# ibm-granite/dolomite-engine

Hardware: NVIDIA H100
Metric: tokens_per_sec (higher is better)
Workload: dtype bf16

## Files before the change

### dolomite_engine_b200/csrc/attention_bwd.cu

```cuda
#include "attention_common.cuh"
#include "../../include/dolomite_b200.h"

using namespace dolo;

namespace {

struct BwdParams {
    const float* lse;
    const float* delta;
    __nv_bfloat16* dqkv;
    int64_t row_stride;
    const int32_t* cu_seqlens;
    int n_docs;
    int64_t T;
    int n_groups, q_per_group, n_heads;
    float scale, scale_log2;
    int head_chunk;
    int head_chunk_q;
    int n_tile_slots;
    AttnDropout drop;
    const float* alibi_slopes;
};

constexpr int DELTA_TOK = 8;
__global__ void __launch_bounds__(256)
    attn_delta_kernel(const uint4* __restrict__ dout, const uint4* __restrict__ out, float* __restrict__ delta, int64_t T,
                      int n_heads, int vec_per_head) {
    extern __shared__ float part[];
    const int64_t t0 = int64_t(blockIdx.x) * DELTA_TOK;
    const int ntok = (T - t0) < DELTA_TOK ? int(T - t0) : DELTA_TOK;
    const int vec_per_tok = n_heads * vec_per_head;
    const int total = ntok * vec_per_tok;
    const uint4* a = dout + t0 * vec_per_tok;
    const uint4* b = out + t0 * vec_per_tok;
    for (int i = threadIdx.x; i < total; i += blockDim.x) {
        const uint4 x = __ldg(a + i), y = __ldg(b + i);
        float s = bf16_lo(x.x) * bf16_lo(y.x) + bf16_hi(x.x) * bf16_hi(y.x);
        s += bf16_lo(x.y) * bf16_lo(y.y) + bf16_hi(x.y) * bf16_hi(y.y);
        s += bf16_lo(x.z) * bf16_lo(y.z) + bf16_hi(x.z) * bf16_hi(y.z);
        s += bf16_lo(x.w) * bf16_lo(y.w) + bf16_hi(x.w) * bf16_hi(y.w);
        part[i] = s;
    }
    __syncthreads();
    for (int i = threadIdx.x; i < n_heads * DELTA_TOK; i += blockDim.x) {
        const int h = i / DELTA_TOK, tl = i - h * DELTA_TOK;
        if (tl < ntok) {
            const float* p = part + tl * vec_per_tok + h * vec_per_head;
            float s = 0.f;
            for (int k = 0; k < vec_per_head; ++k) s += p[k];
            delta[int64_t(h) * T + t0 + tl] = s;
        }
    }
}

constexpr int ATT_BWD_THREADS = 384;
constexpr int ATT_PRODUCER_REGS = 24;
constexpr int ATT_CONSUMER_REGS = 240;
static_assert(ATT_PRODUCER_REGS * 128 + 2 * ATT_CONSUMER_REGS * 128 <= 65536, "register file exceeded");

constexpr int BWD_QT = 64;

__device__ __forceinline__ void opaque(uint32_t& x) { asm volatile("" : "+r"(x)); }
__device__ __forceinline__ void mbar_spin(uint64_t* bar, uint32_t parity) {
    asm volatile("{\n\t.reg .pred P1;\n\tWAIT_%=:\n\tmbarrier.try_wait.parity.shared::cta.b64 P1, [%0], %1;\n\t@!P1 bra WAIT_%=;\n\t}"
                 ::"r"(smem_u32(bar)), "r"(parity)
                 : "memory");
}
__device__ __forceinline__ void mbar_arrive_lane0(uint64_t* bar, int lane) {
    asm volatile("{\n\t.reg .pred p;\n\tsetp.eq.s32 p, %1, 0;\n\t@p mbarrier.arrive.shared::cta.b64 _, [%0];\n\t}" ::"r"(smem_u32(bar)),
                 "r"(lane)
                 : "memory");
}
constexpr int QDO_STAGES = 4;

template <bool ALIBI, bool MASK>
__device__ __forceinline__ void bwd_p_ds(float (&st)[BWD_QT / 2], float (&dpt)[BWD_QT / 2], const float* ls, const float* ds,
                                         const BwdParams& p, const TileLoc& loc, int q0, int wc, const int (&kr)[2], int head,
                                         uint32_t head_key, bool drop) {
    const float slope = ALIBI ? __ldg(p.alibi_slopes + head) : 0.f;
#pragma unroll
    for (int h = 0; h < 2; ++h) {
        const float bias_r = ALIBI ? attn_alibi_bias(slope, kr[h]) * ATT_LOG2E : 0.f;
#pragma unroll
        for (int b = 0; b < BWD_QT / 8; ++b) {
            const float2 l = *reinterpret_cast<const float2*>(ls + 8 * b + wc);
            const float2 d = *reinterpret_cast<const float2*>(ds + 8 * b + wc);
            const float lse_c[2] = {l.x, l.y}, del_c[2] = {d.x, d.y};
#pragma unroll
            for (int e = 0; e < 2; ++e) {
                const int q = q0 + 8 * b + wc + e;
                const int i = 4 * b + 2 * h + e;
                const bool ok = !MASK || (q >= kr[h] && q < loc.doc_len);
                float pr;
                if constexpr (ALIBI)
                    pr = ok ? fast_exp2(fmaf(st[i], p.scale_log2, bias_r) - lse_c[e]) : 0.f;
                else
                    pr = ok ? fast_exp2(fmaf(st[i], p.scale_log2, -lse_c[e])) : 0.f;
                float dp = dpt[i];
                if (drop) {
                    const float z = attn_drop_scale(p.drop, head_key, loc.doc_start + q, loc.doc_start + kr[h]);
                    dp *= z;
                    st[i] = pr * z;
                } else {
                    st[i] = pr;
                }
                dpt[i] = p.scale * pr * (dp - del_c[e]);
            }
        }
    }
}

template <int HD, bool ALIBI>
__global__ void __launch_bounds__(ATT_BWD_THREADS, 1)
    attn_bwd_kernel(const __grid_constant__ CUtensorMap tq64, const __grid_constant__ CUtensorMap tqR,
                    const __grid_constant__ CUtensorMap to64, const __grid_constant__ CUtensorMap toR, const BwdParams p) {
    using CH = HeadChunks<HD>;
    constexpr int KV_BYTES = CH::tile_bytes(ATT_TILE);
    constexpr int QT_BYTES = CH::tile_bytes(BWD_QT);

    int cta_tile, group;
    attn_cta_order(p.head_chunk, p.n_tile_slots, cta_tile, group);
    const TileLoc loc = locate_tile(p.cu_seqlens, p.n_docs, cta_tile);
    if (!loc.valid) return;
    const int k0 = loc.tile * ATT_TILE;
    const int i0 = k0 / BWD_QT;
    const int n_qt = (loc.doc_len + BWD_QT - 1) / BWD_QT;
    const int n_i = n_qt - i0;
    const int n_steps = n_i * p.q_per_group;
    const int k_col = (group * (p.q_per_group + 2) + p.q_per_group) * HD;
    const int v_col = k_col + HD;

    extern __shared__ uint8_t smem_raw[];
    uint8_t* smem = smem_align_1024(smem_raw);
    uint8_t* sK = smem;
    uint8_t* sV = sK + KV_BYTES;
    uint8_t* sQ = sV + KV_BYTES;
    uint8_t* sO = sQ + QDO_STAGES * QT_BYTES;
    float* sL = reinterpret_cast<float*>(sO + QDO_STAGES * QT_BYTES);
    uint64_t* bars = reinterpret_cast<uint64_t*>(sL + QDO_STAGES * 2 * BWD_QT);
    uint64_t* kv_full = bars;
    uint64_t* qd_full = bars + 1;
    uint64_t* qd_empty = bars + 1 + QDO_STAGES;

    const int wg = threadIdx.x >> 7, warp = threadIdx.x >> 5, lane = threadIdx.x & 31;
    const float log2e = 1.4426950408889634f;

    if (threadIdx.x == 0) {
        tma_prefetch_desc(&tq64);
        tma_prefetch_desc(&to64);
        if (CH::REM > 0) {
            tma_prefetch_desc(&tqR);
            tma_prefetch_desc(&toR);
        }
        mbar_init(kv_full, 1);
        for (int i = 0; i < QDO_STAGES; ++i) {
            mbar_init(&qd_full[i], 1 + 32);
            mbar_init(&qd_empty[i], 8);
        }
        mbar_fence_init();
        mbar_expect_tx(kv_full, 2 * KV_BYTES);
        tma_load_chunked<HD, ATT_TILE>(sK, &tq64, &tqR, kv_full, k_col, loc.doc_start + k0);
        tma_load_chunked<HD, ATT_TILE>(sV, &tq64, &tqR, kv_full, v_col, loc.doc_start + k0);
    }
    __syncthreads();

    if (wg == 0) {
        setmaxnreg_dec<ATT_PRODUCER_REGS>();
        if (warp == 0) {
            if (elect_one()) {
                int s = 0;
                uint32_t ph = 0;
                for (int n = 0; n < n_steps; ++n) {
                    const int hl = n / n_i, qi = i0 + n % n_i;
                    const int q_col = (group * (p.q_per_group + 2) + hl) * HD;
                    mbar_wait(&qd_empty[s], ph ^ 1, 32);
                    mbar_expect_tx(&qd_full[s], 2 * QT_BYTES);
                    tma_load_chunked<HD, BWD_QT>(sQ + s * QT_BYTES, &tq64, &tqR, &qd_full[s], q_col,
                                                 loc.doc_start + qi * BWD_QT);
                    tma_load_chunked<HD, BWD_QT>(sO + s * QT_BYTES, &to64, &toR, &qd_full[s],
                                                 (group * p.q_per_group + hl) * HD, loc.doc_start + qi * BWD_QT);
                    if (++s == QDO_STAGES) s = 0, ph ^= 1;
                }
            }
        } else if (warp == 1) {
            int s = 0;
            uint32_t ph = 0;
            for (int n = 0; n < n_steps; ++n) {
                const int hl = n / n_i, qi = i0 + n % n_i;
                const int64_t row0 = int64_t(group * p.q_per_group + hl) * p.T + loc.doc_start;
                mbar_wait(&qd_empty[s], ph ^ 1, 33);
                float* ls = sL + s * 2 * BWD_QT;
#pragma unroll
                for (int r = lane; r < BWD_QT; r += 32) {
                    const int q = qi * BWD_QT + r;
                    ls[r] = q < loc.doc_len ? __ldg(p.lse + row0 + q) * log2e : 0.f;
                    ls[BWD_QT + r] = q < loc.doc_len ? __ldg(p.delta + row0 + q) : 0.f;
                }
                mbar_arrive(&qd_full[s]);
                if (++s == QDO_STAGES) s = 0, ph ^= 1;
            }
        }
        return;
    }

    setmaxnreg_inc<ATT_CONSUMER_REGS>();
    const int cw = wg - 1;
    const int n_steps_u = __shfl_sync(0xffffffffu, n_steps, 0);
    const int wr = (warp & 3) * 16 + (lane >> 2);
    const int wc = 2 * (lane & 3);
    const int kr[2] = {k0 + cw * 64 + wr, k0 + cw * 64 + wr + 8};
    const bool drop = p.drop.threshold != 0;
    const uint32_t sk0 = smem_u32(sK), sv0 = smem_u32(sV);

    float dv[HD / 2], dk[HD / 2];
#pragma unroll
    for (int i = 0; i < HD / 2; ++i) dv[i] = dk[i] = 0.f;
    float st[BWD_QT / 2], dpt[BWD_QT / 2];

    auto issue_ss = [&](int s) {
        const uint32_t sq = smem_u32(sQ + s * QT_BYTES), so = smem_u32(sO + s * QT_BYTES);
        uint32_t sk = sk0, sv = sv0;
        opaque(sk), opaque(sv);
        wgmma_fence();
#pragma unroll
        for (int c = 0; c < CH::NCHUNK; ++c) {
            const int w = CH::width(c);
            const uint32_t krow = CH::offset(c, ATT_TILE) + cw * 64 * 2 * w;
#pragma unroll
            for (int k = 0; k < w / 16; ++k) {
                wgmma_ss<BWD_QT, 0, 0>(st, chunk_desc_kmajor(sk + krow, w, k), chunk_desc_kmajor(sq + CH::offset(c, BWD_QT), w, k),
                                       (c != 0 || k != 0) ? 1u : 0u);
                wgmma_ss<BWD_QT, 0, 0>(dpt, chunk_desc_kmajor(sv + krow, w, k), chunk_desc_kmajor(so + CH::offset(c, BWD_QT), w, k),
                                       (c != 0 || k != 0) ? 1u : 0u);
            }
        }
        wgmma_commit();
    };

    mbar_spin(kv_full, 0);
    int s = 0;
    uint32_t ph = 0;
    for (int n = 0; n < n_steps_u; ++n) {
        const int hl = n / n_i, qi = i0 + n % n_i;
        const int head = group * p.q_per_group + hl;
        const int q0 = qi * BWD_QT;
        const uint32_t head_key = dropout_head_key(uint32_t(head), p.drop.key0, p.drop.key1);
        mbar_spin(&qd_full[s], ph);
        issue_ss(s);
        wgmma_wait<0>();
        reg_fence<BWD_QT / 2>(st);
        reg_fence<BWD_QT / 2>(dpt);

        const float* ls = sL + s * 2 * BWD_QT;
        if (qi <= i0 + cw || (qi + 1) * BWD_QT > loc.doc_len)
            bwd_p_ds<ALIBI, true>(st, dpt, ls, ls + BWD_QT, p, loc, q0, wc, kr, head, head_key, drop);
        else
            bwd_p_ds<ALIBI, false>(st, dpt, ls, ls + BWD_QT, p, loc, q0, wc, kr, head, head_key, drop);
        uint32_t pa[BWD_QT / 16][4], da[BWD_QT / 16][4];
#pragma unroll
        for (int kk = 0; kk < BWD_QT / 16; ++kk) {
            acc_to_a_frag(st, kk, pa[kk]);
            acc_to_a_frag(dpt, kk, da[kk]);
        }

        uint32_t sq = smem_u32(sQ + s * QT_BYTES), so = smem_u32(sO + s * QT_BYTES);
        opaque(sq), opaque(so);
        wgmma_fence();
#pragma unroll
        for (int c = 0; c < CH::NCHUNK; ++c) {
#pragma unroll
            for (int kk = 0; kk < BWD_QT / 16; ++kk) {
                if (CH::width(c) == 64) {
                    wgmma_rs<64, 1>(dv + CH::col(c) / 2, pa[kk], chunk_desc_mnmajor(so + CH::offset(c, BWD_QT), 64, kk), 1u);
                    wgmma_rs<64, 1>(dk + CH::col(c) / 2, da[kk], chunk_desc_mnmajor(sq + CH::offset(c, BWD_QT), 64, kk), 1u);
                } else {
                    constexpr int R = CH::REM ? CH::REM : 16;
                    wgmma_rs<R, 1>(dv + CH::col(c) / 2, pa[kk], chunk_desc_mnmajor(so + CH::offset(c, BWD_QT), R, kk), 1u);
                    wgmma_rs<R, 1>(dk + CH::col(c) / 2, da[kk], chunk_desc_mnmajor(sq + CH::offset(c, BWD_QT), R, kk), 1u);
                }
            }
        }
        wgmma_commit();
        wgmma_wait<0>();
        reg_fence<HD / 2>(dv);
        reg_fence<HD / 2>(dk);
        __syncwarp();
        mbar_arrive_lane0(&qd_empty[s], lane);
        if (++s == QDO_STAGES) s = 0, ph ^= 1;
    }

#pragma unroll
    for (int h = 0; h < 2; ++h) {
        if (kr[h] >= loc.doc_len) continue;
        __nv_bfloat16* row = p.dqkv + (loc.doc_start + int64_t(kr[h])) * p.row_stride;
#pragma unroll
        for (int b = 0; b < HD / 8; ++b) {
            *reinterpret_cast<uint32_t*>(row + k_col + 8 * b + wc) = pack_bf16(dk[4 * b + 2 * h], dk[4 * b + 2 * h + 1]);
            *reinterpret_cast<uint32_t*>(row + v_col + 8 * b + wc) = pack_bf16(dv[4 * b + 2 * h], dv[4 * b + 2 * h + 1]);
        }
    }
}

template <int HD, bool ALIBI>
int launch_bwd(const void* dout, const void* qkv, int64_t row_stride, const BwdParams& p, cudaStream_t st) {
    using CH = HeadChunks<HD>;
    CUtensorMap tq64, tqR, to64, toR;
    int rc = attn_make_maps<HD>(qkv, row_stride, p.T, &tq64, &tqR);
    if (rc) return rc;
    rc = attn_make_maps<HD>(dout, int64_t(p.n_heads) * HD, p.T, &to64, &toR);
    if (rc) return rc;
    constexpr int smem_bytes = 1024 + 2 * CH::tile_bytes(ATT_TILE) + 2 * QDO_STAGES * CH::tile_bytes(BWD_QT) +
                               QDO_STAGES * 2 * BWD_QT * 4 + 128;
    static_assert(smem_bytes <= 232448, "attention backward shared memory budget exceeded");
    auto kern = attn_bwd_kernel<HD, ALIBI>;
    static bool attr_set = false;
    if (!attr_set) {
        DOLO_CUDA_OK(cudaFuncSetAttribute(kern, cudaFuncAttributeMaxDynamicSharedMemorySize, smem_bytes));
        attr_set = true;
    }
    const int64_t max_tiles = (p.T + ATT_TILE - 1) / ATT_TILE + p.n_docs;
    DOLO_REQUIRE(max_tiles == p.n_tile_slots && max_tiles * p.n_groups < (1ll << 31), "attn_bwd: grid too large");
    dim3 grid((unsigned)(max_tiles * p.n_groups));
    kern<<<grid, ATT_BWD_THREADS, smem_bytes, st>>>(tq64, tqR, to64, toR, p);
    DOLO_LAUNCH_OK("attn_varlen_bwd");
    return DOLO_OK;
}

constexpr int DQ_KT = 64;
constexpr int KV_STAGES = 4;

template <bool ALIBI, bool MASK>
__device__ __forceinline__ void dq_ds(float (&sc)[DQ_KT / 2], const float (&dp)[DQ_KT / 2], const BwdParams& p,
                                      const TileLoc& loc, int j, int wc, const int (&qr)[2], const float (&lse_r)[2],
                                      const float (&del_r)[2], float slope, uint32_t head_key, bool drop) {
    if constexpr (ALIBI) {
#pragma unroll
        for (int b = 0; b < DQ_KT / 8; ++b)
#pragma unroll
            for (int e = 0; e < 2; ++e) {
                const int k = j * DQ_KT + 8 * b + wc + e;
                const float bl = attn_alibi_bias(slope, k) * ATT_LOG2E;
#pragma unroll
                for (int h = 0; h < 2; ++h) {
                    const int i = 4 * b + 2 * h + e;
                    const bool ok = !MASK || (k <= qr[h] && qr[h] < loc.doc_len);
                    const float pr = ok ? fast_exp2(fmaf(sc[i], p.scale_log2, bl) - lse_r[h]) : 0.f;
                    float d = dp[i];
                    if (drop) d *= attn_drop_scale(p.drop, head_key, loc.doc_start + qr[h], loc.doc_start + k);
                    sc[i] = p.scale * pr * (d - del_r[h]);
                }
            }
    } else {
#pragma unroll
        for (int h = 0; h < 2; ++h)
#pragma unroll
            for (int b = 0; b < DQ_KT / 8; ++b)
#pragma unroll
                for (int e = 0; e < 2; ++e) {
                    const int k = j * DQ_KT + 8 * b + wc + e;
                    const int i = 4 * b + 2 * h + e;
                    const bool ok = !MASK || (k <= qr[h] && qr[h] < loc.doc_len);
                    const float pr = ok ? fast_exp2(fmaf(sc[i], p.scale_log2, -lse_r[h])) : 0.f;
                    float d = dp[i];
                    if (drop) d *= attn_drop_scale(p.drop, head_key, loc.doc_start + qr[h], loc.doc_start + k);
                    sc[i] = p.scale * pr * (d - del_r[h]);
                }
    }
}

template <int HD, bool ALIBI>
__global__ void __launch_bounds__(ATT_BWD_THREADS, 1)
    attn_dq_kernel(const __grid_constant__ CUtensorMap tq64, const __grid_constant__ CUtensorMap tqR,
                   const __grid_constant__ CUtensorMap to64, const __grid_constant__ CUtensorMap toR, const BwdParams p) {
    using CH = HeadChunks<HD>;
    constexpr int Q_BYTES = CH::tile_bytes(ATT_TILE);
// ... 304 lines not shown
```

### dolomite_engine_b200/csrc/attention_common.cuh

```cuda
#pragma once
#include "common.cuh"
#include "wgmma.cuh"
#include "../../include/dolomite_b200.h"

namespace dolo {

constexpr int ATT_TILE = 128;

template <int HD>
struct HeadChunks {
    static_assert(HD % 16 == 0 && HD >= 16 && HD <= 128, "head_dim must be a multiple of 16 in [16, 128]");
    static constexpr int NC64 = HD / 64;
    static constexpr int REM = HD % 64;
    static_assert(REM == 0 || REM == 16 || REM == 32, "head_dim % 64 must be 0, 16 or 32");
    static constexpr int NCHUNK = NC64 + (REM ? 1 : 0);
    __host__ __device__ static constexpr int width(int c) { return c < NC64 ? 64 : REM; }
    __host__ __device__ static constexpr int col(int c) { return c * 64; }
    __host__ __device__ static constexpr int offset(int c, int rows) { return c * rows * 128; }
    __host__ __device__ static constexpr int tile_bytes(int rows) { return rows * HD * 2; }
};

__host__ __device__ constexpr uint32_t chunk_layout_type(int w) { return w == 64 ? 1u : (w == 32 ? 2u : 3u); }

__device__ __forceinline__ uint64_t chunk_desc_kmajor(uint32_t chunk_saddr, int w, int k16) {
    return gmma_desc(chunk_saddr + k16 * 32, 16, 16 * w, chunk_layout_type(w));
}
__device__ __forceinline__ uint64_t chunk_desc_mnmajor(uint32_t chunk_saddr, int w, int k16) {
    return gmma_desc(chunk_saddr + k16 * 32 * w, 16 * w, 16 * w, chunk_layout_type(w));
}

template <int HD, int ROWS>
__device__ __forceinline__ void tma_load_chunked(uint8_t* dst, const CUtensorMap* m64, const CUtensorMap* mR, uint64_t* bar,
                                                 int col0, int row0) {
    using CH = HeadChunks<HD>;
#pragma unroll
    for (int c = 0; c < CH::NCHUNK; ++c)
#pragma unroll
        for (int h = 0; h < ROWS / 64; ++h)
            tma_load_2d(dst + CH::offset(c, ROWS) + h * 64 * 2 * CH::width(c), c < CH::NC64 ? m64 : mR, bar,
                        col0 + CH::col(c), row0 + h * 64);
}

template <int HD>
int attn_make_maps(const void* base, int64_t ld, int64_t rows, CUtensorMap* m64, CUtensorMap* mR) {
    using CH = HeadChunks<HD>;
    uint64_t dims[2] = {uint64_t(ld), uint64_t(rows)};
    uint64_t strides[2] = {2, uint64_t(ld) * 2};
    uint32_t box[2] = {64, 64};
    int rc;
    if (CH::NC64 > 0) {
        rc = dolo_make_tmap(m64, base, 2, 2, dims, strides, box, DOLO_SW_128);
        if (rc) return rc;
    }
    if (CH::REM > 0) {
        box[0] = CH::REM;
        rc = dolo_make_tmap(mR, base, 2, 2, dims, strides, box, CH::REM == 32 ? DOLO_SW_64 : DOLO_SW_32);
        if (rc) return rc;
    }
    if (CH::NC64 == 0) *m64 = *mR;
    if (CH::REM == 0) *mR = *m64;
    return DOLO_OK;
}

struct AttnDropout {
    uint32_t threshold;
    float keep_scale;
    uint32_t key0, key1;
};
__device__ __forceinline__ float attn_drop_scale(const AttnDropout& d, uint32_t head_key, int q_tok, int k_tok) {
    return dropout_hash_qk(uint32_t(q_tok), uint32_t(k_tok), head_key) >= d.threshold ? d.keep_scale : 0.f;
}

__device__ __forceinline__ float attn_alibi_bias(float slope, int kpos) {
    return __bfloat162float(__float2bfloat16_rn(slope * float(kpos)));
}
constexpr float ATT_LOG2E = 1.4426950408889634f;
constexpr float ATT_LN2 = 0.6931471805599453f;

__device__ __forceinline__ void attn_cta_order(int chunk, int n_tile_slots, int& tile, int& head) {
    const int id = int(blockIdx.x);
    if (chunk <= 0) {
        tile = id % n_tile_slots;
        head = id / n_tile_slots;
        return;
    }
    const int per = n_tile_slots * chunk;
    const int c = id / per, r = id - c * per;
    tile = r / chunk;
    head = c * chunk + (r - tile * chunk);
}
inline int attn_head_chunk(int option, int n, int align) {
    if (option <= 0 || n <= 0) return 0;
    if (align < 1 || n % align != 0) align = 1;
    int best = 0;
    for (int c = align; c <= n; c += align)
        if (n % c == 0 && c <= (option > align ? option : align)) best = c;
    return best > 0 ? best : n;
}

struct TileLoc {
    int doc_start;
    int doc_len;
    int tile;
    bool valid;
};
__device__ __forceinline__ TileLoc locate_tile(const int32_t* __restrict__ cu, int n_docs, int ti) {
    TileLoc r{0, 0, 0, false};
    int acc = 0;
    for (int d = 0; d < n_docs; ++d) {
        const int s = cu[d], e = cu[d + 1];
        const int nt = (e - s + ATT_TILE - 1) / ATT_TILE;
        if (ti < acc + nt) {
            r.doc_start = s;
            r.doc_len = e - s;
            r.tile = ti - acc;
            r.valid = true;
            return r;
        }
        acc += nt;
    }
    return r;
}

}
```

### dolomite_engine_b200/csrc/attention_fwd.cu

```cuda
#include "attention_common.cuh"
#include "../../include/dolomite_b200.h"

using namespace dolo;

namespace {

constexpr int FWD_THREADS = 256;
constexpr int KV_STAGES = 2;

struct FwdParams {
    __nv_bfloat16* out;
    float* lse;
    const int32_t* cu_seqlens;
    int n_docs;
    int64_t T;
    int n_groups, q_per_group;
    int n_heads;
    float scale_log2;
    float scale;
    AttnDropout drop;
    int head_chunk;
    int n_tile_slots;
    const float* alibi_slopes;
};

template <int HD, bool ALIBI>
__global__ void __launch_bounds__(FWD_THREADS, 1)
    attn_fwd_kernel(const __grid_constant__ CUtensorMap tmap64, const __grid_constant__ CUtensorMap tmapR,
                    const FwdParams p) {
    using CH = HeadChunks<HD>;
    constexpr int TILE_BYTES = CH::tile_bytes(ATT_TILE);

    int ti, head;
    attn_cta_order(p.head_chunk, p.n_tile_slots, ti, head);
    ti = p.n_tile_slots - 1 - ti;
    const TileLoc loc = locate_tile(p.cu_seqlens, p.n_docs, ti);
    if (!loc.valid) return;
    const int group = head / p.q_per_group, slot = head % p.q_per_group;
    const int q_col = (group * (p.q_per_group + 2) + slot) * HD;
    const int k_col = (group * (p.q_per_group + 2) + p.q_per_group) * HD;
    const int v_col = k_col + HD;
    const int q0 = loc.tile * ATT_TILE;
    const int n_kv = loc.tile + 1;

    extern __shared__ uint8_t smem_raw[];
    uint8_t* smem = smem_align_1024(smem_raw);
    uint8_t* sQ = smem;
    uint8_t* sK = sQ + TILE_BYTES;
    uint8_t* sV = sK + KV_STAGES * TILE_BYTES;
    uint64_t* bars = reinterpret_cast<uint64_t*>(sV + KV_STAGES * TILE_BYTES);
    uint64_t* q_full = bars;
    uint64_t* kv_full = bars + 1;
    uint64_t* kv_empty = bars + 3;

    const int wg = threadIdx.x >> 7, warp = threadIdx.x >> 5, lane = threadIdx.x & 31;

    auto load_kv = [&](int j, int s) {
        mbar_expect_tx(&kv_full[s], 2 * TILE_BYTES);
        tma_load_chunked<HD, ATT_TILE>(sK + s * TILE_BYTES, &tmap64, &tmapR, &kv_full[s], k_col, loc.doc_start + j * ATT_TILE);
        tma_load_chunked<HD, ATT_TILE>(sV + s * TILE_BYTES, &tmap64, &tmapR, &kv_full[s], v_col, loc.doc_start + j * ATT_TILE);
    };
    if (threadIdx.x == 0) {
        if (CH::NC64 > 0) tma_prefetch_desc(&tmap64);
        if (CH::REM > 0) tma_prefetch_desc(&tmapR);
        mbar_init(q_full, 1);
        for (int i = 0; i < KV_STAGES; ++i) {
            mbar_init(&kv_full[i], 1);
            mbar_init(&kv_empty[i], FWD_THREADS / 32);
        }
        mbar_fence_init();
        mbar_expect_tx(q_full, TILE_BYTES);
        tma_load_chunked<HD, ATT_TILE>(sQ, &tmap64, &tmapR, q_full, q_col, loc.doc_start + q0);
        for (int j = 0; j < KV_STAGES && j < n_kv; ++j) load_kv(j, j);
    }
    __syncthreads();

    const int wr = (warp & 3) * 16 + (lane >> 2);
    const int wc = 2 * (lane & 3);
    const int qr[2] = {q0 + wg * 64 + wr, q0 + wg * 64 + wr + 8};
    const bool drop = p.drop.threshold != 0;
    const uint32_t head_key = dropout_head_key(uint32_t(head), p.drop.key0, p.drop.key1);
    const uint32_t sq = smem_u32(sQ);

    float o[HD / 2];
#pragma unroll
    for (int i = 0; i < HD / 2; ++i) o[i] = 0.f;
    float m_run[2] = {-INFINITY, -INFINITY}, l_run[2] = {0.f, 0.f};
    const float slope = ALIBI ? __ldg(p.alibi_slopes + head) : 0.f;

    mbar_wait(q_full, 0, 10);
    for (int j = 0; j < n_kv; ++j) {
        const int s = j & (KV_STAGES - 1);
        mbar_wait(&kv_full[s], (j / KV_STAGES) & 1, 11);
        const uint32_t sk = smem_u32(sK + s * TILE_BYTES), sv = smem_u32(sV + s * TILE_BYTES);
        float sc[ATT_TILE / 2];
        wgmma_fence();
#pragma unroll
        for (int c = 0; c < CH::NCHUNK; ++c) {
            const int w = CH::width(c);
#pragma unroll
            for (int k = 0; k < w / 16; ++k)
                wgmma_ss<ATT_TILE, 0, 0>(sc, chunk_desc_kmajor(sq + CH::offset(c, ATT_TILE) + wg * 64 * 2 * w, w, k),
                                         chunk_desc_kmajor(sk + CH::offset(c, ATT_TILE), w, k), (c != 0 || k != 0) ? 1u : 0u);
        }
        wgmma_commit();
        wgmma_wait<0>();
        reg_fence<ATT_TILE / 2>(sc);

        const bool diag = j == loc.tile;
        const int kbase = j * ATT_TILE + wc;
        if constexpr (ALIBI) {
#pragma unroll
            for (int b = 0; b < ATT_TILE / 8; ++b)
#pragma unroll
                for (int e = 0; e < 2; ++e) {
                    const float bl = attn_alibi_bias(slope, kbase + 8 * b + e) * ATT_LOG2E;
                    sc[4 * b + e] = fmaf(sc[4 * b + e], p.scale_log2, bl);
                    sc[4 * b + 2 + e] = fmaf(sc[4 * b + 2 + e], p.scale_log2, bl);
                }
        }
#pragma unroll
        for (int h = 0; h < 2; ++h) {
            float mx = m_run[h];
#pragma unroll
            for (int b = 0; b < ATT_TILE / 8; ++b)
#pragma unroll
                for (int e = 0; e < 2; ++e) {
                    float& x = sc[4 * b + 2 * h + e];
                    if (diag && kbase + 8 * b + e > qr[h]) x = -INFINITY;
                    mx = fmaxf(mx, x);
                }
            mx = fmaxf(mx, __shfl_xor_sync(0xffffffffu, mx, 1));
            mx = fmaxf(mx, __shfl_xor_sync(0xffffffffu, mx, 2));
            const float corr = ALIBI ? fast_exp2(m_run[h] - mx) : fast_exp2((m_run[h] - mx) * p.scale_log2);
            const float neg_m = ALIBI ? -mx : -mx * p.scale_log2;
            float lsum = 0.f;
#pragma unroll
            for (int b = 0; b < ATT_TILE / 8; ++b)
#pragma unroll
                for (int e = 0; e < 2; ++e) {
                    float& x = sc[4 * b + 2 * h + e];
                    float pr = ALIBI ? fast_exp2(x + neg_m) : fast_exp2(fmaf(x, p.scale_log2, neg_m));
                    lsum += pr;
                    if (drop)
                        pr *= attn_drop_scale(p.drop, head_key, loc.doc_start + qr[h], loc.doc_start + kbase + 8 * b + e);
                    x = pr;
                }
            l_run[h] = l_run[h] * corr + lsum;
            m_run[h] = mx;
#pragma unroll
            for (int b = 0; b < HD / 8; ++b) {
                o[4 * b + 2 * h] *= corr;
                o[4 * b + 2 * h + 1] *= corr;
            }
        }
        uint32_t pa[ATT_TILE / 16][4];
#pragma unroll
        for (int kk = 0; kk < ATT_TILE / 16; ++kk) acc_to_a_frag(sc, kk, pa[kk]);

        wgmma_fence();
#pragma unroll
        for (int c = 0; c < CH::NCHUNK; ++c) {
#pragma unroll
            for (int kk = 0; kk < ATT_TILE / 16; ++kk) {
                if (CH::width(c) == 64)
                    wgmma_rs<64, 1>(o + CH::col(c) / 2, pa[kk], chunk_desc_mnmajor(sv + CH::offset(c, ATT_TILE), 64, kk), 1u);
                else
                    wgmma_rs<(CH::REM ? CH::REM : 16), 1>(o + CH::col(c) / 2, pa[kk],
                                                          chunk_desc_mnmajor(sv + CH::offset(c, ATT_TILE), CH::REM, kk), 1u);
            }
        }
        wgmma_commit();
        wgmma_wait<0>();
        reg_fence<HD / 2>(o);
        if (lane == 0) mbar_arrive(&kv_empty[s]);
        if (threadIdx.x == 0 && j + KV_STAGES < n_kv) {
            mbar_wait(&kv_empty[s], (j / KV_STAGES) & 1, 12);
            load_kv(j + KV_STAGES, s);
        }
        __syncwarp();
    }

#pragma unroll
    for (int h = 0; h < 2; ++h) {
        float l = l_run[h];
        l += __shfl_xor_sync(0xffffffffu, l, 1);
        l += __shfl_xor_sync(0xffffffffu, l, 2);
        if (qr[h] >= loc.doc_len) continue;
        const float inv_l = l > 0.f ? 1.f / l : 0.f;
        const int64_t row = loc.doc_start + qr[h];
        __nv_bfloat16* orow = p.out + row * (int64_t(p.n_heads) * HD) + int64_t(head) * HD + wc;
#pragma unroll
        for (int b = 0; b < HD / 8; ++b)
            *reinterpret_cast<uint32_t*>(orow + 8 * b) = pack_bf16(o[4 * b + 2 * h] * inv_l, o[4 * b + 2 * h + 1] * inv_l);
        if ((lane & 3) == 0)
            p.lse[int64_t(head) * p.T + row] = (ALIBI ? m_run[h] * ATT_LN2 : m_run[h] * p.scale) + logf(l);
    }
}

template <int HD, bool ALIBI>
int launch_fwd(const void* qkv, int64_t row_stride, const FwdParams& p, cudaStream_t st) {
    using CH = HeadChunks<HD>;
    CUtensorMap t64, tR;
    int rc = attn_make_maps<HD>(qkv, row_stride, p.T, &t64, &tR);
    if (rc) return rc;
    constexpr int smem_bytes = 1024 + (1 + 2 * KV_STAGES) * CH::tile_bytes(ATT_TILE) + 128;
    static_assert(smem_bytes <= 232448, "attention forward shared memory budget exceeded");
    auto kern = attn_fwd_kernel<HD, ALIBI>;
    static bool attr_set = false;
    if (!attr_set) {
        DOLO_CUDA_OK(cudaFuncSetAttribute(kern, cudaFuncAttributeMaxDynamicSharedMemorySize, smem_bytes));
        attr_set = true;
    }
    const int64_t max_tiles = (p.T + ATT_TILE - 1) / ATT_TILE + p.n_docs;
    DOLO_REQUIRE(max_tiles == p.n_tile_slots && max_tiles * p.n_heads < (1ll << 31), "attn_fwd: grid too large");
    dim3 grid((unsigned)(max_tiles * p.n_heads));
    kern<<<grid, FWD_THREADS, smem_bytes, st>>>(t64, tR, p);
    DOLO_LAUNCH_OK("attn_varlen_fwd");
    return DOLO_OK;
}

}

uint32_t dolo_dropout_threshold(float p);

extern "C" int dolomite_b200_attn_varlen_fwd(const void* qkv, int64_t row_stride, void* out, float* lse,
                                             const int32_t* cu_seqlens, int n_docs, int64_t T, int max_seqlen,
                                             int n_groups, int q_per_group, int head_dim, float softmax_scale,
                                             void* stream) {
    return dolomite_b200_attn_varlen_fwd_dropout(qkv, row_stride, out, lse, cu_seqlens, n_docs, T, max_seqlen, n_groups,
                                                 q_per_group, head_dim, softmax_scale, 0.f, 0, 0, stream);
}

namespace {

int attn_fwd(const void* qkv, int64_t row_stride, void* out, float* lse, const int32_t* cu_seqlens, int n_docs, int64_t T,
             int n_groups, int q_per_group, int head_dim, float softmax_scale, float dropout_p, uint32_t key0, uint32_t key1,
             const float* alibi_slopes, void* stream) {
    DOLO_REQUIRE(dropout_p >= 0.f && dropout_p < 1.f, "attn_fwd: dropout_p=%f must be in [0, 1)", double(dropout_p));
    DOLO_REQUIRE(n_docs >= 0 && T >= 0, "attn_fwd: negative sizes");
    if (T == 0 || n_docs == 0) return DOLO_OK;
    DOLO_REQUIRE(n_groups > 0 && q_per_group > 0, "attn_fwd: bad head grouping");
    DOLO_REQUIRE(row_stride % 8 == 0 && (reinterpret_cast<uintptr_t>(qkv) & 15) == 0, "attn_fwd: qkv alignment");
    DOLO_REQUIRE(int64_t(n_groups) * (q_per_group + 2) * head_dim <= row_stride, "attn_fwd: slot layout exceeds row");
    DOLO_REQUIRE(T < (1ll << 31), "attn_fwd: T too large");
    FwdParams p;
    p.out = static_cast<__nv_bfloat16*>(out);
    p.lse = lse;
    p.cu_seqlens = cu_seqlens;
    p.n_docs = n_docs;
    p.T = T;
    p.n_groups = n_groups;
    p.q_per_group = q_per_group;
    p.n_heads = n_groups * q_per_group;
    p.scale = softmax_scale;
    p.scale_log2 = softmax_scale * 1.4426950408889634f;
    p.drop.threshold = dolo_dropout_threshold(dropout_p);
    p.drop.keep_scale = 1.f / (1.f - dropout_p);
    p.drop.key0 = key0;
    p.drop.key1 = key1;
    p.n_tile_slots = int((T + ATT_TILE - 1) / ATT_TILE + n_docs);
    p.head_chunk = attn_head_chunk(dolo_option_attn_head_fastest(), p.n_heads, q_per_group);
    if (p.head_chunk > 0 && T * int64_t(n_groups) * head_dim * 4 <= (24ll << 20)) p.head_chunk = p.n_heads;
    p.alibi_slopes = alibi_slopes;
    cudaStream_t st = static_cast<cudaStream_t>(stream);
    const bool ab = alibi_slopes != nullptr;
    switch (head_dim) {
        case 16: return ab ? launch_fwd<16, true>(qkv, row_stride, p, st) : launch_fwd<16, false>(qkv, row_stride, p, st);
        case 32: return ab ? launch_fwd<32, true>(qkv, row_stride, p, st) : launch_fwd<32, false>(qkv, row_stride, p, st);
        case 64: return ab ? launch_fwd<64, true>(qkv, row_stride, p, st) : launch_fwd<64, false>(qkv, row_stride, p, st);
        case 80: return ab ? launch_fwd<80, true>(qkv, row_stride, p, st) : launch_fwd<80, false>(qkv, row_stride, p, st);
        case 96: return ab ? launch_fwd<96, true>(qkv, row_stride, p, st) : launch_fwd<96, false>(qkv, row_stride, p, st);
        case 128: return ab ? launch_fwd<128, true>(qkv, row_stride, p, st) : launch_fwd<128, false>(qkv, row_stride, p, st);
        default: return dolo_set_error("attn_fwd: unsupported head_dim %d (supported: 16,32,64,80,96,128)", head_dim);
    }
}

}

extern "C" int dolomite_b200_attn_varlen_fwd_dropout(const void* qkv, int64_t row_stride, void* out, float* lse,
                                                     const int32_t* cu_seqlens, int n_docs, int64_t T, int max_seqlen,
                                                     int n_groups, int q_per_group, int head_dim, float softmax_scale,
                                                     float dropout_p, uint32_t key0, uint32_t key1, void* stream) {
    (void)max_seqlen;
    return attn_fwd(qkv, row_stride, out, lse, cu_seqlens, n_docs, T, n_groups, q_per_group, head_dim, softmax_scale,
                    dropout_p, key0, key1, nullptr, stream);
}

extern "C" int dolomite_b200_attn_varlen_fwd_alibi(const void* qkv, int64_t row_stride, void* out, float* lse,
                                                   const int32_t* cu_seqlens, int n_docs, int64_t T, int max_seqlen,
                                                   int n_groups, int q_per_group, int head_dim, float softmax_scale,
                                                   float dropout_p, uint32_t key0, uint32_t key1,
                                                   const float* alibi_slopes, void* stream) {
    (void)max_seqlen;
    DOLO_REQUIRE(alibi_slopes != nullptr, "attn_fwd_alibi: alibi_slopes is null");
    return attn_fwd(qkv, row_stride, out, lse, cu_seqlens, n_docs, T, n_groups, q_per_group, head_dim, softmax_scale,
                    dropout_p, key0, key1, alibi_slopes, stream);
}
```

Baseline: 18280.

## Warp-specialize attention forward with producer warp and ping-pong consumer warpgroups

Restructures the forward attention kernel into a producer warpgroup issuing TMA K/V loads and two consumer warpgroups. The consumers overlap the next QK^T wgmma with the current softmax and use named barriers to alternate tensor-core turns. KV pipeline stages go from 2 to 3 or 4 depending on head dim, and the diagonal mask is only applied on the last step. The aim is to hide softmax and load latency behind matrix math, at the cost of more shared memory, register reallocation and more complex synchronisation.

```diff
diff --git a/dolomite_engine_b200/csrc/attention_bwd.cu b/dolomite_engine_b200/csrc/attention_bwd.cu
--- a/dolomite_engine_b200/csrc/attention_bwd.cu
+++ b/dolomite_engine_b200/csrc/attention_bwd.cu
@@ -53,24 +53,10 @@
     }
 }
 
-constexpr int ATT_BWD_THREADS = 384;
-constexpr int ATT_PRODUCER_REGS = 24;
-constexpr int ATT_CONSUMER_REGS = 240;
-static_assert(ATT_PRODUCER_REGS * 128 + 2 * ATT_CONSUMER_REGS * 128 <= 65536, "register file exceeded");
+constexpr int ATT_BWD_THREADS = ATT_WS_THREADS;
 
 constexpr int BWD_QT = 64;
 
-__device__ __forceinline__ void opaque(uint32_t& x) { asm volatile("" : "+r"(x)); }
-__device__ __forceinline__ void mbar_spin(uint64_t* bar, uint32_t parity) {
-    asm volatile("{\n\t.reg .pred P1;\n\tWAIT_%=:\n\tmbarrier.try_wait.parity.shared::cta.b64 P1, [%0], %1;\n\t@!P1 bra WAIT_%=;\n\t}"
-                 ::"r"(smem_u32(bar)), "r"(parity)
-                 : "memory");
-}
-__device__ __forceinline__ void mbar_arrive_lane0(uint64_t* bar, int lane) {
-    asm volatile("{\n\t.reg .pred p;\n\tsetp.eq.s32 p, %1, 0;\n\t@p mbarrier.arrive.shared::cta.b64 _, [%0];\n\t}" ::"r"(smem_u32(bar)),
-                 "r"(lane)
-                 : "memory");
-}
 constexpr int QDO_STAGES = 4;
 
 template <bool ALIBI, bool MASK>
diff --git a/dolomite_engine_b200/csrc/attention_common.cuh b/dolomite_engine_b200/csrc/attention_common.cuh
--- a/dolomite_engine_b200/csrc/attention_common.cuh
+++ b/dolomite_engine_b200/csrc/attention_common.cuh
@@ -98,6 +98,32 @@
     return best > 0 ? best : n;
 }
 
+constexpr int ATT_WS_THREADS = 384;
+constexpr int ATT_PRODUCER_REGS = 24;
+constexpr int ATT_CONSUMER_REGS = 240;
+static_assert(ATT_PRODUCER_REGS * 128 + 2 * ATT_CONSUMER_REGS * 128 <= 65536, "register file exceeded");
+
+__device__ __forceinline__ void opaque(uint32_t& x) { asm volatile("" : "+r"(x)); }
+__device__ __forceinline__ void mbar_spin(uint64_t* bar, uint32_t parity) {
+    asm volatile("{\n\t.reg .pred P1;\n\tWAIT_%=:\n\tmbarrier.try_wait.parity.shared::cta.b64 P1, [%0], %1;\n\t@!P1 bra WAIT_%=;\n\t}"
+                 ::"r"(smem_u32(bar)), "r"(parity)
+                 : "memory");
+}
+__device__ __forceinline__ void mbar_arrive_lane0(uint64_t* bar, int lane) {
+    asm volatile("{\n\t.reg .pred p;\n\tsetp.eq.s32 p, %1, 0;\n\t@p mbarrier.arrive.shared::cta.b64 _, [%0];\n\t}" ::"r"(smem_u32(bar)),
+                 "r"(lane)
+                 : "memory");
+}
+
+__device__ __forceinline__ void named_bar_sync_if(bool c, uint32_t id, uint32_t n) {
+    asm volatile("{\n\t.reg .pred p;\n\tsetp.ne.b32 p, %0, 0;\n\t@p bar.sync %1, %2;\n\t}" ::"r"(int(c)), "r"(id), "r"(n)
+                 : "memory");
+}
+__device__ __forceinline__ void named_bar_arrive_if(bool c, uint32_t id, uint32_t n) {
+    asm volatile("{\n\t.reg .pred p;\n\tsetp.ne.b32 p, %0, 0;\n\t@p bar.arrive %1, %2;\n\t}" ::"r"(int(c)), "r"(id), "r"(n)
+                 : "memory");
+}
+
 struct TileLoc {
     int doc_start;
     int doc_len;
diff --git a/dolomite_engine_b200/csrc/attention_fwd.cu b/dolomite_engine_b200/csrc/attention_fwd.cu
--- a/dolomite_engine_b200/csrc/attention_fwd.cu
+++ b/dolomite_engine_b200/csrc/attention_fwd.cu
@@ -1,3 +1,5 @@
+#include <type_traits>
+
 #include "attention_common.cuh"
 #include "../../include/dolomite_b200.h"
 
@@ -5,8 +7,15 @@
 
 namespace {
 
-constexpr int FWD_THREADS = 256;
-constexpr int KV_STAGES = 2;
+constexpr int FWD_THREADS = ATT_WS_THREADS;
+template <int HD>
+constexpr int fwd_kv_stages() {
+    return HD <= 96 ? 4 : 3;
+}
+template <int HD>
+constexpr int fwd_smem_bytes() {
+    return 1024 + (1 + 2 * fwd_kv_stages<HD>()) * HeadChunks<HD>::tile_bytes(ATT_TILE) + 128;
+}
 
 struct FwdParams {
     __nv_bfloat16* out;
@@ -24,24 +33,65 @@
     const float* alibi_slopes;
 };
 
+template <bool ALIBI, bool MASK>
+__device__ __forceinline__ void fwd_softmax(float (&sc)[ATT_TILE / 2], float (&m_run)[2], float (&l_run)[2], float (&corr)[2],
+                                            const FwdParams& p, int kbase, const int (&qr)[2], float slope, int doc_start,
+                                            uint32_t head_key, bool drop) {
+    if constexpr (ALIBI) {
+#pragma unroll
+        for (int b = 0; b < ATT_TILE / 8; ++b)
+#pragma unroll
+            for (int e = 0; e < 2; ++e) {
+                const float bl = attn_alibi_bias(slope, kbase + 8 * b + e) * ATT_LOG2E;
+                sc[4 * b + e] = fmaf(sc[4 * b + e], p.scale_log2, bl);
+                sc[4 * b + 2 + e] = fmaf(sc[4 * b + 2 + e], p.scale_log2, bl);
+            }
+    }
+#pragma unroll
+    for (int h = 0; h < 2; ++h) {
+        float mx = m_run[h];
+#pragma unroll
+        for (int b = 0; b < ATT_TILE / 8; ++b)
+#pragma unroll
+            for (int e = 0; e < 2; ++e) {
+                float& x = sc[4 * b + 2 * h + e];
+                if (MASK && kbase + 8 * b + e > qr[h]) x = -INFINITY;
+                mx = fmaxf(mx, x);
+            }
+        mx = fmaxf(mx, __shfl_xor_sync(0xffffffffu, mx, 1));
+        mx = fmaxf(mx, __shfl_xor_sync(0xffffffffu, mx, 2));
+        corr[h] = ALIBI ? fast_exp2(m_run[h] - mx) : fast_exp2((m_run[h] - mx) * p.scale_log2);
+        const float neg_m = ALIBI ? -mx : -mx * p.scale_log2;
+        float lsum = 0.f;
+#pragma unroll
+        for (int b = 0; b < ATT_TILE / 8; ++b)
+#pragma unroll
+            for (int e = 0; e < 2; ++e) {
+                float& x = sc[4 * b + 2 * h + e];
+                float pr = ALIBI ? fast_exp2(x + neg_m) : fast_exp2(fmaf(x, p.scale_log2, neg_m));
+                lsum += pr;
+                if (drop)
+                    pr *= attn_drop_scale(p.drop, head_key, doc_start + qr[h], doc_start + kbase + 8 * b + e);
+                x = pr;
+            }
+        l_run[h] = l_run[h] * corr[h] + lsum;
+        m_run[h] = mx;
+    }
+}
+
 template <int HD, bool ALIBI>
 __global__ void __launch_bounds__(FWD_THREADS, 1)
     attn_fwd_kernel(const __grid_constant__ CUtensorMap tmap64, const __grid_constant__ CUtensorMap tmapR,
                     const FwdParams p) {
     using CH = HeadChunks<HD>;
     constexpr int TILE_BYTES = CH::tile_bytes(ATT_TILE);
+    constexpr int KV_STAGES = fwd_kv_stages<HD>();
 
     int ti, head;
     attn_cta_order(p.head_chunk, p.n_tile_slots, ti, head);
     ti = p.n_tile_slots - 1 - ti;
-    const TileLoc loc = locate_tile(p.cu_seqlens, p.n_docs, ti);
+    TileLoc loc = locate_tile(p.cu_seqlens, p.n_docs, ti);
     if (!loc.valid) return;
-    const int group = head / p.q_per_group, slot = head % p.q_per_group;
-    const int q_col = (group * (p.q_per_group + 2) + slot) * HD;
-    const int k_col = (group * (p.q_per_group + 2) + p.q_per_group) * HD;
-    const int v_col = k_col + HD;
-    const int q0 = loc.tile * ATT_TILE;
-    const int n_kv = loc.tile + 1;
 
     extern __shared__ uint8_t smem_raw[];
     uint8_t* smem = smem_align_1024(smem_raw);
@@ -51,36 +101,61 @@
     uint64_t* bars = reinterpret_cast<uint64_t*>(sV + KV_STAGES * TILE_BYTES);
     uint64_t* q_full = bars;
     uint64_t* kv_full = bars + 1;
-    uint64_t* kv_empty = bars + 3;
+    uint64_t* kv_empty = bars + 1 + KV_STAGES;
+    __shared__ int4 tile_info;
 
     const int wg = threadIdx.x >> 7, warp = threadIdx.x >> 5, lane = threadIdx.x & 31;
 
-    auto load_kv = [&](int j, int s) {
-        mbar_expect_tx(&kv_full[s], 2 * TILE_BYTES);
-        tma_load_chunked<HD, ATT_TILE>(sK + s * TILE_BYTES, &tmap64, &tmapR, &kv_full[s], k_col, loc.doc_start + j * ATT_TILE);
-        tma_load_chunked<HD, ATT_TILE>(sV + s * TILE_BYTES, &tmap64, &tmapR, &kv_full[s], v_col, loc.doc_start + j * ATT_TILE);
-    };
     if (threadIdx.x == 0) {
         if (CH::NC64 > 0) tma_prefetch_desc(&tmap64);
         if (CH::REM > 0) tma_prefetch_desc(&tmapR);
         mbar_init(q_full, 1);
         for (int i = 0; i < KV_STAGES; ++i) {
             mbar_init(&kv_full[i], 1);
-            mbar_init(&kv_empty[i], FWD_THREADS / 32);
+            mbar_init(&kv_empty[i], 8);
         }
         mbar_fence_init();
+        const int q_col = (head / p.q_per_group * (p.q_per_group + 2) + head % p.q_per_group) * HD;
         mbar_expect_tx(q_full, TILE_BYTES);
-        tma_load_chunked<HD, ATT_TILE>(sQ, &tmap64, &tmapR, q_full, q_col, loc.doc_start + q0);
-        for (int j = 0; j < KV_STAGES && j < n_kv; ++j) load_kv(j, j);
+        tma_load_chunked<HD, ATT_TILE>(sQ, &tmap64, &tmapR, q_full, q_col, loc.doc_start + loc.tile * ATT_TILE);
+        tile_info = make_int4(head, loc.doc_start, loc.doc_len, loc.tile);
     }
     __syncthreads();
-
+    {
+        const int4 t = tile_info;
+        head = t.x, loc.doc_start = t.y, loc.doc_len = t.z, loc.tile = t.w;
+    }
+    const int k_col = (head / p.q_per_group * (p.q_per_group + 2) + p.q_per_group) * HD;
+    const int v_col = k_col + HD;
+    const int q0 = loc.tile * ATT_TILE;
+    const int n_kv = loc.tile + 1;
+
+    if (wg == 0) {
+        setmaxnreg_dec<ATT_PRODUCER_REGS>();
+        if (warp == 0 && elect_one()) {
+            int s = 0;
+            uint32_t ph = 0;
+            for (int j = 0; j < n_kv; ++j) {
+                mbar_wait(&kv_empty[s], ph ^ 1, 12);
+                mbar_expect_tx(&kv_full[s], 2 * TILE_BYTES);
+                tma_load_chunked<HD, ATT_TILE>(sK + s * TILE_BYTES, &tmap64, &tmapR, &kv_full[s], k_col,
+                                               loc.doc_start + j * ATT_TILE);
+                tma_load_chunked<HD, ATT_TILE>(sV + s * TILE_BYTES, &tmap64, &tmapR, &kv_full[s], v_col,
+                                               loc.doc_start + j * ATT_TILE);
+                if (++s == KV_STAGES) s = 0, ph ^= 1;
+            }
+        }
+        return;
+    }
+
+    setmaxnreg_inc<ATT_CONSUMER_REGS>();
+    const int cw = wg - 1;
+    const int n_kv_u = __shfl_sync(0xffffffffu, n_kv, 0);
     const int wr = (warp & 3) * 16 + (lane >> 2);
     const int wc = 2 * (lane & 3);
-    const int qr[2] = {q0 + wg * 64 + wr, q0 + wg * 64 + wr + 8};
+    const int qr[2] = {q0 + cw * 64 + wr, q0 + cw * 64 + wr + 8};
     const bool drop = p.drop.threshold != 0;
     const uint32_t head_key = dropout_head_key(uint32_t(head), p.drop.key0, p.drop.key1);
-    const uint32_t sq = smem_u32(sQ);
 
     float o[HD / 2];
 #pragma unroll
@@ -88,76 +163,59 @@
     float m_run[2] = {-INFINITY, -INFINITY}, l_run[2] = {0.f, 0.f};
     const float slope = ALIBI ? __ldg(p.alibi_slopes + head) : 0.f;
 
-    mbar_wait(q_full, 0, 10);
-    for (int j = 0; j < n_kv; ++j) {
-        const int s = j & (KV_STAGES - 1);
-        mbar_wait(&kv_full[s], (j / KV_STAGES) & 1, 11);
-        const uint32_t sk = smem_u32(sK + s * TILE_BYTES), sv = smem_u32(sV + s * TILE_BYTES);
-        float sc[ATT_TILE / 2];
+    auto issue_s = [&](float (&sc)[ATT_TILE / 2], int s) {
+        uint32_t sq = smem_u32(sQ), sk = smem_u32(sK + s * TILE_BYTES);
+        opaque(sq), opaque(sk);
         wgmma_fence();
 #pragma unroll
         for (int c = 0; c < CH::NCHUNK; ++c) {
             const int w = CH::width(c);
 #pragma unroll
             for (int k = 0; k < w / 16; ++k)
-                wgmma_ss<ATT_TILE, 0, 0>(sc, chunk_desc_kmajor(sq + CH::offset(c, ATT_TILE) + wg * 64 * 2 * w, w, k),
+                wgmma_ss<ATT_TILE, 0, 0>(sc, chunk_desc_kmajor(sq + CH::offset(c, ATT_TILE) + cw * 64 * 2 * w, w, k),
                                          chunk_desc_kmajor(sk + CH::offset(c, ATT_TILE), w, k), (c != 0 || k != 0) ? 1u : 0u);
         }
         wgmma_commit();
+    };
+
+    auto turn_begin = [&](bool not_first) { named_bar_sync_if(not_first || cw == 1, 1 + cw, 256); };
+    auto turn_end = [&](bool not_last) { named_bar_arrive_if(not_last || cw == 0, 2 - cw, 256); };
+
+    float sc[ATT_TILE / 2];
+    int s = 0;
+    uint32_t ph = 0;
+    int s_prev = 0;
+    auto step = [&](auto more_c, int j) {
+        constexpr bool MORE = decltype(more_c)::value;
+        const int s1 = s + 1 == KV_STAGES ? 0 : s + 1;
+        const uint32_t ph1 = s1 == 0 ? ph ^ 1 : ph;
+        float corr[2];
+        fwd_softmax<ALIBI, !MORE>(sc, m_run, l_run, corr, p, j * ATT_TILE + wc, qr, slope, loc.doc_start, head_key, drop);
+
         wgmma_wait<0>();
-        reg_fence<ATT_TILE / 2>(sc);
-
-        const bool diag = j == loc.tile;
-        const int kbase = j * ATT_TILE + wc;
-        if constexpr (ALIBI) {
-#pragma unroll
-            for (int b = 0; b < ATT_TILE / 8; ++b)
-#pragma unroll
-                for (int e = 0; e < 2; ++e) {
-                    const float bl = attn_alibi_bias(slope, kbase + 8 * b + e) * ATT_LOG2E;
-                    sc[4 * b + e] = fmaf(sc[4 * b + e], p.scale_log2, bl);
-                    sc[4 * b + 2 + e] = fmaf(sc[4 * b + 2 + e], p.scale_log2, bl);
-                }
-        }
-#pragma unroll
-        for (int h = 0; h < 2; ++h) {
-            float mx = m_run[h];
-#pragma unroll
-            for (int b = 0; b < ATT_TILE / 8; ++b)
-#pragma unroll
-                for (int e = 0; e < 2; ++e) {
-                    float& x = sc[4 * b + 2 * h + e];
-                    if (diag && kbase + 8 * b + e > qr[h]) x = -INFINITY;
-                    mx = fmaxf(mx, x);
-                }
-            mx = fmaxf(mx, __shfl_xor_sync(0xffffffffu, mx, 1));
-            mx = fmaxf(mx, __shfl_xor_sync(0xffffffffu, mx, 2));
-            const float corr = ALIBI ? fast_exp2(m_run[h] - mx) : fast_exp2((m_run[h] - mx) * p.scale_log2);
-            const float neg_m = ALIBI ? -mx : -mx * p.scale_log2;
-            float lsum = 0.f;
-#pragma unroll
-            for (int b = 0; b < ATT_TILE / 8; ++b)
-#pragma unroll
-                for (int e = 0; e < 2; ++e) {
-                    float& x = sc[4 * b + 2 * h + e];
-                    float pr = ALIBI ? fast_exp2(x + neg_m) : fast_exp2(fmaf(x, p.scale_log2, neg_m));
-                    lsum += pr;
-                    if (drop)
-                        pr *= attn_drop_scale(p.drop, head_key, loc.doc_start + qr[h], loc.doc_start + kbase + 8 * b + e);
-                    x = pr;
-                }
-            l_run[h] = l_run[h] * corr + lsum;
-            m_run[h] = mx;
+        reg_fence<HD / 2>(o);
+        if (j > 0) {
+            __syncwarp();
+            mbar_arrive_lane0(&kv_empty[s_prev], lane);
+        }
+#pragma unroll
+        for (int h = 0; h < 2; ++h)
 #pragma unroll
             for (int b = 0; b < HD / 8; ++b) {
-                o[4 * b + 2 * h] *= corr;
-                o[4 * b + 2 * h + 1] *= corr;
-            }
-        }
+                o[4 * b + 2 * h] *= corr[h];
+                o[4 * b + 2 * h + 1] *= corr[h];
+            }
         uint32_t pa[ATT_TILE / 16][4];
 #pragma unroll
         for (int kk = 0; kk < ATT_TILE / 16; ++kk) acc_to_a_frag(sc, kk, pa[kk]);
 
+        turn_begin(true);
+        if constexpr (MORE) {
+            mbar_spin(&kv_full[s1], ph1);
+            issue_s(sc, s1);
+        }
+        uint32_t sv = smem_u32(sV + s * TILE_BYTES);
+        opaque(sv);
         wgmma_fence();
 #pragma unroll
         for (int c = 0; c < CH::NCHUNK; ++c) {
@@ -171,15 +229,34 @@
             }
         }
         wgmma_commit();
-        wgmma_wait<0>();
-        reg_fence<HD / 2>(o);
-        if (lane == 0) mbar_arrive(&kv_empty[s]);
-        if (threadIdx.x == 0 && j + KV_STAGES < n_kv) {
-            mbar_wait(&kv_empty[s], (j / KV_STAGES) & 1, 12);
-            load_kv(j + KV_STAGES, s);
-        }
-        __syncwarp();
-    }
+        turn_end(MORE);
+        if constexpr (MORE) {
+            wgmma_wait<1>();
+            reg_fence<ATT_TILE / 2>(sc);
+        }
+        s_prev = s, s = s1, ph = ph1;
+    };
+
+    mbar_spin(q_full, 0);
+    mbar_spin(&kv_full[0], 0);
+    turn_begin(false);
+    issue_s(sc, 0);
+    turn_end(true);
+    wgmma_wait<0>();
+    reg_fence<ATT_TILE / 2>(sc);
+    int j = 0;
+    for (; j + 2 < n_kv_u; j += 2) {
+        step(std::true_type{}, j);
+        step(std::true_type{}, j + 1);
+    }
+    if (j + 1 < n_kv_u) {
+        step(std::true_type{}, j);
+        step(std::false_type{}, j + 1);
+    } else {
+        step(std::false_type{}, j);
+    }
+    wgmma_wait<0>();
+    reg_fence<HD / 2>(o);
 
 #pragma unroll
     for (int h = 0; h < 2; ++h) {
@@ -194,17 +271,16 @@
         for (int b = 0; b < HD / 8; ++b)
             *reinterpret_cast<uint32_t*>(orow + 8 * b) = pack_bf16(o[4 * b + 2 * h] * inv_l, o[4 * b + 2 * h + 1] * inv_l);
         if ((lane & 3) == 0)
-            p.lse[int64_t(head) * p.T + row] = (ALIBI ? m_run[h] * ATT_LN2 : m_run[h] * p.scale) + logf(l);
+            p.lse[int64_t(head) * p.T + row] = ALIBI ? __fmul_rn(m_run[h], ATT_LN2) + logf(l) : fmaf(m_run[h], p.scale, logf(l));
     }
 }
 
 template <int HD, bool ALIBI>
 int launch_fwd(const void* qkv, int64_t row_stride, const FwdParams& p, cudaStream_t st) {
-    using CH = HeadChunks<HD>;
     CUtensorMap t64, tR;
     int rc = attn_make_maps<HD>(qkv, row_stride, p.T, &t64, &tR);
     if (rc) return rc;
-    constexpr int smem_bytes = 1024 + (1 + 2 * KV_STAGES) * CH::tile_bytes(ATT_TILE) + 128;
+    constexpr int smem_bytes = fwd_smem_bytes<HD>();
     static_assert(smem_bytes <= 232448, "attention forward shared memory budget exceeded");
     auto kern = attn_fwd_kernel<HD, ALIBI>;
     static bool attr_set = false;
```

After: 18390, median of 6. No clear change (+0.6%).
